# schreibfaul1/ESP32-Opus-Player

Hardware: AMD Instinct MI355X
Metric: decoded 48 kHz stereo frames/sec/GPU (x real-time); HBM GB/s vs roofline (higher is better)
Workload: dtype int32 fixed-point (int16/int32 with 64-bit products); 1 GPU; celt_fb_stereo_64k; streams_per_gpu=65536

## Files before the change

### esp32-opus-player_amd/csrc/og_celt_split.hpp

```cpp
#pragma once
#include <stddef.h>
#include "og_celt.hpp"

#undef OG_SYNC
#define OG_SYNC() OG_LSYNC()

namespace og {

constexpr int REC_BAND_WORDS = 4;
constexpr int REC_MAX_LEAVES = NBANDS * 2 * 16;
constexpr int REC_MAX_WORDS = NBANDS * (REC_BAND_WORDS + 2 * 33) + 3 * NBANDS + 1;

enum {
    RF_SILENCE = 1, RF_TRANSIENT = 2, RF_LM_SHIFT = 2 , RF_STEREO = 16, RF_SPREAD_SHIFT = 5 ,
    RF_DUAL = 128, RF_ANTI_COLLAPSE = 256, RF_RC_ERROR = 512, RF_TELL_OVERFLOW = 1024,
    RF_SKIP = 2048,
    RF_BAD_CELT = 4096
};
enum {
    BW_SIGN0 = 1, BW_SIGN1 = 2, BW_INV = 4, BW_SIGN = 8, BW_MID_FIRST = 16, BW_SWAP = 32,
    BW_THETA0 = 64, BW_THETA1 = 128,
    BW_TF_SHIFT = 8 , BW_FOLD0_SHIFT = 11 , BW_FOLD1_SHIFT = 16 ,
    BW_HAS_LOW = 1 << 21, BW_DUAL = 1 << 22, BW_DUAL_END = 1 << 23, BW_STEREO = 1 << 24,
    BW_DUAL_PRE = 1 << 25
};
enum {
    JW_NPVQ_SHIFT = 5 , JW_FIRST_SHIFT = 10 , JW_NEED_LOW = 1 << 20,
    LW_OFF_SHIFT = 8 , LW_B_SHIFT = 12 , LW_N_SHIFT = 16
};

struct SilkHandoff {
    alignas(128) i16 pcm[1920];
    u32 valid;
    u32 storage, end_offs, end_window;
    i32 nend_bits, nbits_total;
    u32 offs, rng, val, ext;
    i32 rem, error;
};
static_assert(sizeof(SilkHandoff) % 128 == 0 && offsetof(SilkHandoff, pcm) == 0, "handoff alignment");

struct ParseRec {
    i32 ret;
    u32 rng_final;
    u32 flags;
    i32 intensity, pf_pitch, pf_gain, pf_tapset, start;
    i32 n_leaves, n_words;
    u32 need_norm;
    i32 n_coef;
    i32 reserved[4];
    i16 bandE[2 * NBANDS];
    i16 pulses[NBANDS];
    u16 band_w[NBANDS];
    i8 tf_res[NBANDS];
    i8 pad[256 - 64 - 4 * NBANDS - 2 * NBANDS - 2 * NBANDS - NBANDS];
    struct Leaf {
        u32 idx;
        u32 geom;
        u32 aux;
        u32 pad;
    } leaf[REC_MAX_LEAVES];
    u32 words[(REC_MAX_WORDS + 64) / 64 * 64];
    i32 work_pulses[NBANDS];
    i32 work_pad[32 - NBANDS];
};
static_assert(offsetof(ParseRec, leaf) % 16 == 0 && offsetof(ParseRec, words) % 16 == 0 && offsetof(ParseRec, work_pulses) % 16 == 0 &&
              offsetof(ParseRec, work_pad) == offsetof(ParseRec, work_pulses) + 4 * NBANDS && NBANDS + 3 <= 32, "16-byte stores into the record");
static_assert(sizeof(ParseRec) % 16 == 0, "record alignment");

constexpr int FAST_MAX_LEAVES = 416;

#ifndef OG_PL_LANES
#define OG_PL_LANES (OG_NLANES >= 32 ? 32 : OG_NLANES)
#endif
#ifndef OG_PL_WAVES
#define OG_PL_WAVES 1
#endif
#ifdef OG_HOST_EMUL
#define OG_PWAVE 0
#define OG_PCOL OG_LANE
#else
#define OG_PWAVE ((int)(threadIdx.x >> 6))
#define OG_PCOL ((int)(threadIdx.x & 63))
#endif
#define OG_PL_FRAMES (OG_PL_LANES * OG_PL_WAVES)
struct ParseLds {
    i8 fine_quant[NBANDS][OG_PL_LANES];
    i8 tf_prio[NBANDS][OG_PL_LANES];
    union {
        i16 bandE[2 * NBANDS][OG_PL_LANES];
        struct {
            i16 offsets[NBANDS][OG_PL_LANES];
            u32 bw[NBANDS][OG_PL_LANES];
        } al;
        i32 stack[5][6][OG_PL_LANES];
    } u;
#ifdef OG_PL_PAD
    u8 pad_experiment[OG_PL_PAD];
#endif
};
#ifdef OG_PARSE_DYN_LDS
extern __shared__ __attribute__((aligned(16))) unsigned char og_dyn_lds[];
#define PLs (reinterpret_cast<ParseLds *>(og_dyn_lds))
#else
OG_LDS ParseLds PLs[OG_PL_WAVES];
#endif
#define PL PLs[OG_PWAVE]

struct ParseTabLds {
    i16 eband[NBANDS + 1], logn[NBANDS];
    u16 pulse_idx[105];
    u32 pulse_v[392];
    u8 pulse_bits[392], band_alloc[231], pulse_caps[168], log2_frac[24], eprob[336];
};
#ifdef OG_PARSE_DYN_LDS
#define PT (*reinterpret_cast<ParseTabLds *>(og_dyn_lds + sizeof(ParseLds) * OG_PL_WAVES))
#define OG_PARSE_LDS_BYTES (sizeof(ParseLds) * OG_PL_WAVES + sizeof(ParseTabLds))
#else
OG_LDS ParseTabLds PT;
#define OG_PARSE_LDS_BYTES 0
#endif
struct RomLds {
    static OG_MEMBER i32 eband(int i) { return PT.eband[i]; }
    static OG_MEMBER i32 logn(int i) { return PT.logn[i]; }
    static OG_MEMBER i32 pulse_idx(int i) { return PT.pulse_idx[i]; }
    static OG_MEMBER i32 pulse_bits(int i) { return PT.pulse_bits[i]; }
    static OG_MEMBER i32 band_alloc(int i) { return PT.band_alloc[i]; }
    static OG_MEMBER i32 pulse_caps(int i) { return PT.pulse_caps[i]; }
    static OG_MEMBER i32 log2_frac(int i) { return PT.log2_frac[i]; }
    static OG_MEMBER i32 eprob(int i) { return PT.eprob[i]; }
};
OG_DEV void parse_tables_load() {
    OG_FOR_LANES(i, NBANDS + 1) PT.eband[i] = rom_eband[i];
    OG_FOR_LANES(i, NBANDS) PT.logn[i] = rom_logn[i];
    OG_FOR_LANES(i, 105) PT.pulse_idx[i] = rom_pulse_idx[i];
    OG_FOR_LANES(i, 392) PT.pulse_bits[i] = rom_pulse_bits[i];
    OG_FOR_LANES(i, 392) PT.pulse_v[i] = rom_pulse_v[i];
    OG_FOR_LANES(i, 231) PT.band_alloc[i] = rom_band_alloc[i];
    OG_FOR_LANES(i, 168) PT.pulse_caps[i] = rom_pulse_caps[i];
    OG_FOR_LANES(i, 24) PT.log2_frac[i] = rom_log2_frac[i];
    OG_FOR_LANES(i, 336) PT.eprob[i] = rom_eprob[i];
    OG_FULL_SYNC();
}

struct TfResView {
    i8 *p;
    OG_MEMBER operator int() const { return (int)(i8)((u8)*p << 4) >> 4; }
    OG_MEMBER void operator=(int v) const { *p = (i8)((*p & 0xF0) | (v & 15)); }
};
struct FinePrioView {
    i8 *p;
    OG_MEMBER operator int() const { return (*p >> 4) & 1; }
    OG_MEMBER void operator=(int v) const { *p = (i8)((*p & ~0x10) | ((v & 1) << 4)); }
};
struct LaneArr {
    typedef RomLds Rom;
    i32 *pl;
    i16 *rest;
    i16 *pk;
    OG_MEMBER void energies_rest() const {
        for (int i = 0; i < 2 * NBANDS; i += 2)
            *reinterpret_cast<u32 *>(&rest[i]) = (u32)(u16)PL.u.bandE[i][OG_PCOL] | (u32)(u16)PL.u.bandE[i + 1][OG_PCOL] << 16;
        for (int i = 0; i < NBANDS; i++) PL.u.al.offsets[i][OG_PCOL] = 0;
    }
    OG_MEMBER void energies_back() const {
        u32 w[NBANDS];
        for (int i = 0; i < NBANDS; i++) w[i] = *reinterpret_cast<const u32 *>(&rest[2 * i]);
        for (int i = 0; i < NBANDS; i++) {
            PL.u.bandE[2 * i][OG_PCOL] = (i16)(w[i] & 0xffff);
            PL.u.bandE[2 * i + 1][OG_PCOL] = (i16)(w[i] >> 16);
        }
    }
    typedef u16 __attribute__((may_alias)) u16a;
    typedef i32 __attribute__((may_alias)) i32a;
    OG_MEMBER i32 &pulses(int i) const { return pl[i]; }
    OG_MEMBER i32a &alloc_bits(int i) const { return *reinterpret_cast<i32a *>(&PL.u.al.bw[i][OG_PCOL]); }
    OG_MEMBER void pulses_rest(int start, int end) const {
        i32 v[24];
        for (int i = 0; i < 24; i++) v[i] = (i >= start && i < end) ? (i32)PL.u.al.bw[i < NBANDS ? i : 0][OG_PCOL] : 0;
#ifdef OG_HOST_EMUL
        for (int i = 0; i < NBANDS; i++) pl[i] = v[i];
#else
        typedef i32 i32x4 __attribute__((ext_vector_type(4)));
        for (int i = 0; i < 24; i += 4) *reinterpret_cast<i32x4 *>(&pl[i]) = i32x4{v[i], v[i + 1], v[i + 2], v[i + 3]};
#endif
        for (int i = 0; i < NBANDS; i++) pk[i] = (i16)v[i];
    }
    OG_MEMBER i8 &fine_quant(int i) const { return PL.fine_quant[i][OG_PCOL]; }
    OG_MEMBER FinePrioView fine_prio(int i) const { return FinePrioView{&PL.tf_prio[i][OG_PCOL]}; }
    OG_MEMBER TfResView tf_res(int i) const { return TfResView{&PL.tf_prio[i][OG_PCOL]}; }
    OG_MEMBER i16 &offsets(int i) const { return PL.u.al.offsets[i][OG_PCOL]; }
    OG_MEMBER u16a &bits1(int i) const { return reinterpret_cast<u16a *>(&PL.u.al.bw[i][OG_PCOL])[0]; }
    OG_MEMBER u16a &bits2(int i) const { return reinterpret_cast<u16a *>(&PL.u.al.bw[i][OG_PCOL])[1]; }
    OG_MEMBER i16 &bandE(int i) const { return PL.u.bandE[i][OG_PCOL]; }
};

OG_DEV u32 pvq_u_rom(int a, int b) {
    const int lo = a < b ? a : b, hi = a < b ? b : a;
    return rom_pvq_u[lo * ROM_PVQ_COLS + hi];
}

struct RecWriter {
    ParseRec *rec;
    int nw, nl, ncoef = 0;
    int job = 0;
    OG_MEMBER void word(u32 w) {
        if (nw < REC_MAX_WORDS) rec->words[nw] = w;
        nw++;
    }
    OG_MEMBER int reserve() { return nw++; }
    OG_MEMBER void patch(int at, u32 w) {
        if (at < REC_MAX_WORDS) rec->words[at] = w;
    }
    OG_MEMBER void leaf(int x, int N, int K, int B, i32 gain, int off, u32 idx) {
        if (nl < REC_MAX_LEAVES) {
            const u32 geom = (u32)x | (u32)N << 11 | (u32)K << 19 | (u32)(B - 1) << 27;
            const u32 aux = (u32)(gain & 0xffff) | (u32)off << 16 | (u32)job << 20;
#ifdef OG_HOST_EMUL
            rec->leaf[nl].idx = idx; rec->leaf[nl].geom = geom; rec->leaf[nl].aux = aux; rec->leaf[nl].pad = 0;
#else
            typedef u32 u32x4 __attribute__((ext_vector_type(4)));
            *reinterpret_cast<u32x4 *>(&rec->leaf[nl]) = u32x4{idx, geom, aux, 0u};
#endif
        }
        nl++;
        ncoef += N;
    }
    OG_MEMBER int band_begin() { return nw = (nw + 3) & ~3; }
    OG_MEMBER void words4(u32 w0, u32 w1, u32 w2, u32 w3) {
        if (nw + 4 <= REC_MAX_WORDS) {
#ifdef OG_HOST_EMUL
            rec->words[nw] = w0; rec->words[nw + 1] = w1; rec->words[nw + 2] = w2; rec->words[nw + 3] = w3;
#else
            typedef u32 u32x4 __attribute__((ext_vector_type(4)));
            *reinterpret_cast<u32x4 *>(&rec->words[nw]) = u32x4{w0, w1, w2, w3};
#endif
        }
        nw += 4;
    }
};

OG_DEV int parse_tree(RcLane &rc, RecWriter &out, int band, i32 &remaining_bits, int x, int N, i32 b, int B, int LM, i32 gain,
                      int has_low, int silent) {
    int depth = 0, off = 0, n_fill = 0;
    const int jpos = out.reserve(), first_pvq = out.nl;
    for (;;) {
        OG_MARK(41);
        for (;;) {
            if (!(LM != -1 && b > pulse_cache_max<RomLds>(band, LM) + 12 && N > 2)) break;
            const int B0 = B;
            Split sc;
            i32 fill = 0;
            N >>= 1;
            LM -= 1;
            B = (B + 1) >> 1;
            compute_theta<RomLds>(rc, band, 0, 0, remaining_bits, sc, N, b, B, B0, LM, 0, fill);
            i32 delta = sc.delta;
            const int itheta = sc.itheta;
            if (B0 > 1 && (itheta & 0x3fff)) {
                if (itheta > 8192)
                    delta -= delta >> (4 - LM);
                else
                    delta = OG_MIN(0, delta + (N << BITRES >> (5 - LM)));
            }
            const i32 mbits = OG_MAX(0, OG_MIN(b, (b - delta) / 2));
            const i32 sbits = b - mbits;
            remaining_bits -= sc.qalloc;
            const int mid_first = mbits >= sbits;
            const int off_side = off + (B0 >> 1), silent_mid = silent | (itheta == 16384), silent_side = silent | (itheta == 0);
            i32 *F = &PL.u.stack[depth][0][OG_PCOL];
            F[0 * OG_PL_LANES] = x | N << 11 | (LM + 1) << 19 | B << 22 | mid_first << 27 | 1 << 28;
            F[1 * OG_PL_LANES] = mbits;
            F[2 * OG_PL_LANES] = sbits;
            F[3 * OG_PL_LANES] = remaining_bits;
            F[4 * OG_PL_LANES] = itheta | (mid_first ? off_side : off) << 16 | (mid_first ? silent_side : silent_mid) << 24;
            const i32 gain_mid = tr16(mul16_p15(gain, sc.imid)), gain_side = tr16(mul16_p15(gain, sc.iside));
            F[5 * OG_PL_LANES] = (gain_mid & 0xffff) | gain_side << 16;
            depth++;
            if (mid_first) {
                b = mbits;
                gain = gain_mid;
                silent = silent_mid;
            } else {
                x += N;
                b = sbits;
                gain = gain_side;
                off = off_side;
                silent = silent_side;
            }
        }
        {
            OG_MARK(42);
            int q = bits2pulses<RomLds>(band, LM, b), curr_bits = pulses2bits<RomLds>(band, LM, q);
            remaining_bits -= curr_bits;
            while (remaining_bits < 0 && q > 0) {
                remaining_bits += curr_bits;
                q--;
                curr_bits = pulses2bits<RomLds>(band, LM, q);
                remaining_bits -= curr_bits;
            }
            const int K = q ? get_pulses(q) : 0;
            OG_MARK(43);
            if (K)
                out.leaf(x, N, K, B, gain, off, rc_uint(rc, PT.pulse_v[pulse_cache<RomLds>(band, LM) + q]));
            else if (!silent) {
                out.word((u32)off << LW_OFF_SHIFT | (u32)(B - 1) << LW_B_SHIFT | (u32)N << LW_N_SHIFT);
                out.word((u32)x | (u32)(gain & 0xffff) << 11);
                n_fill++;
            }
        }
        OG_MARK(44);
        for (;;) {
            if (depth == 0) {
                OG_MARK(40);
                const int need_low = has_low && n_fill > 0;
                out.patch(jpos, (u32)n_fill | (u32)(out.nl - first_pvq) << JW_NPVQ_SHIFT | (u32)first_pvq << JW_FIRST_SHIFT |
                                    (need_low ? JW_NEED_LOW : 0));
                return need_low;
            }
            i32 *F = &PL.u.stack[depth - 1][0][OG_PCOL];
            const i32 w0 = F[0];
            const int mid_first = (w0 >> 27) & 1, stage = (w0 >> 28) & 3;
            if (stage == 1) {
                i32 mbits = F[1 * OG_PL_LANES], sbits = F[2 * OG_PL_LANES];
                const int itheta = F[4 * OG_PL_LANES] & 0x7fff;
                const i32 rebalance = (mid_first ? mbits : sbits) - (F[3 * OG_PL_LANES] - remaining_bits);
                if (mid_first) {
                    if (rebalance > 3 << BITRES && itheta != 0) sbits += rebalance - (3 << BITRES);
                } else {
                    if (rebalance > 3 << BITRES && itheta != 16384) mbits += rebalance - (3 << BITRES);
                }
                F[0] = (w0 & ~(3 << 28)) | 2 << 28;
                N = (w0 >> 11) & 255;
                LM = ((w0 >> 19) & 7) - 1;
                B = (w0 >> 22) & 31;
                x = (w0 & 2047) + (mid_first ? N : 0);
                b = mid_first ? sbits : mbits;
                gain = mid_first ? F[5 * OG_PL_LANES] >> 16 : (i32)(i16)F[5 * OG_PL_LANES];
                off = (F[4 * OG_PL_LANES] >> 16) & 15;
                silent = (F[4 * OG_PL_LANES] >> 24) & 1;
                break;
            }
            depth--;
        }
    }
}

OG_DEV u32 parse_all_bands(RcLane &rc, RecWriter &out, int start, int end, int C, int N_ch, int shortBlocks, int spread,
                           int dual_stereo, int intensity, i32 total_bits, i32 balance, int LM, int codedBands, int disable_inv) {
    const LaneArr a{out.rec->work_pulses, nullptr, nullptr};
    const int M = 1 << LM, B = shortBlocks ? M : 1;
    const int norm_offset = M * RomLds::eband(start);
    int lowband_offset = 0, update_lowband = 1;
    u32 need_norm = 0;
#ifdef OG_HOST_EMUL
    i32 p4[4] = {0, 0, 0, 0}, n4[4] = {0, 0, 0, 0};
    auto fetch4 = [&](int b, i32 *o) { for (int k = 0; k < 4; k++) o[k] = b + k < NBANDS ? a.pulses(b + k) : 0; };
    fetch4(start & ~3, n4);
#else
    typedef i32 i32x4p __attribute__((ext_vector_type(4)));
    i32x4p p4 = {0, 0, 0, 0}, n4 = *reinterpret_cast<const i32x4p *>(&a.pulses(start & ~3));
#endif
    for (int i = start; i < end; i++) {
        if (i == start || (i & 3) == 0) {
#ifdef OG_HOST_EMUL
            for (int k = 0; k < 4; k++) p4[k] = n4[k];
            fetch4((i & ~3) + 4, n4);
#else
            p4 = n4;
            n4 = *reinterpret_cast<const i32x4p *>(&a.pulses((i & ~3) + 4));
#endif
        }
        const i32 pulses_i = (i & 3) == 0 ? p4[0] : (i & 3) == 1 ? p4[1] : (i & 3) == 2 ? p4[2] : p4[3];
        const int eb0 = M * RomLds::eband(i), N = M * RomLds::eband(i + 1) - eb0;
        const int x = eb0, y = C == 2 ? N_ch + eb0 : -1;
        out.rec->band_w[i] = (u16)OG_MIN(out.band_begin(), REC_MAX_WORDS);
        const i32 tell = (i32)rc_tell_frac(rc);
        if (i != start) balance -= tell;
        i32 remaining_bits = total_bits - tell - 1, b;
        if (i <= codedBands - 1) {
            const i32 curr_balance = balance / OG_MIN(3, codedBands - i);
            b = OG_MAX(0, OG_MIN(16383, OG_MIN(remaining_bits + 1, pulses_i + curr_balance)));
        } else
            b = 0;
        const int tf_change = a.tf_res(i);
        if ((eb0 - N >= M * RomLds::eband(start) || i == start + 1) && (update_lowband || lowband_offset == 0)) lowband_offset = i;
        u32 w0 = (u32)(tf_change + 4) << BW_TF_SHIFT, w1 = (u32)eb0 << 11 | (u32)N << 22;
        int has_low = 0;
        u32 fold_bands = 0;
        if (lowband_offset != 0 && (spread != 3 || B > 1 || tf_change < 0)) {
            const int effective_lowband = OG_MAX(0, M * RomLds::eband(lowband_offset) - norm_offset - N);
            int fold_start = lowband_offset;
            while (M * RomLds::eband(--fold_start) > effective_lowband + norm_offset) {}
            int fold_end = lowband_offset - 1;
            while (++fold_end < i && M * RomLds::eband(fold_end) < effective_lowband + norm_offset + N) {}
            w0 |= BW_HAS_LOW | (u32)fold_start << BW_FOLD0_SHIFT | (u32)fold_end << BW_FOLD1_SHIFT;
            w1 |= (u32)effective_lowband;
            has_low = 1;
            fold_bands = (1u << fold_end) - (1u << fold_start);
        }
        if (dual_stereo) w0 |= BW_DUAL_PRE;
        if (dual_stereo && i == intensity) {
            dual_stereo = 0;
            w0 |= BW_DUAL_END;
        }
        if (dual_stereo) w0 |= BW_DUAL;
        u32 w2 = 0;
        if (N == 1) {
            for (int c = 0; c < (y >= 0 ? 2 : 1); c++) {
                if (remaining_bits >= 1 << BITRES) {
                    if (rc_bits(rc, 1)) w0 |= c ? BW_SIGN1 : BW_SIGN0;
                    remaining_bits -= 1 << BITRES;
                }
            }
            out.words4(w0, w1, 0, 0);
        } else {
            const int stereo = (y >= 0) && !dual_stereo;
            Split sc;
            sc.inv = 0; sc.imid = 0; sc.iside = 0; sc.delta = 0; sc.itheta = 0; sc.qalloc = 0;
            i32 bb = b, fill_unused = 0, mbits = 0, sbits = 0, rebal0 = 0;
            int n2case = 0, swap_c = 0, mid_first = 1, njobs = 1;
            if (stereo) {
                compute_theta<RomLds>(rc, i, intensity, disable_inv, remaining_bits, sc, N, bb, B, B, LM, 1, fill_unused);
                w0 |= BW_STEREO;
                if (sc.itheta == 0) w0 |= BW_THETA0;
                if (sc.itheta == 16384) w0 |= BW_THETA1;
                if (sc.itheta > 8192) w0 |= BW_SWAP;
                if (sc.inv) w0 |= BW_INV;
                w2 = (u32)(sc.imid & 0xffff) | (u32)sc.iside << 16;
                if (N == 2) {
                    n2case = 1;
                    mbits = bb;
                    sbits = 0;
                    if (sc.itheta != 0 && sc.itheta != 16384) sbits = 1 << BITRES;
                    mbits -= sbits;
                    swap_c = sc.itheta > 8192;
                    remaining_bits -= sc.qalloc + sbits;
                    if (sbits && rc_bits(rc, 1)) w0 |= BW_SIGN;
                } else {
                    mbits = OG_MAX(0, OG_MIN(bb, (bb - sc.delta) / 2));
                    sbits = bb - mbits;
                    remaining_bits -= sc.qalloc;
                    rebal0 = remaining_bits;
                    mid_first = mbits >= sbits;
                    njobs = 2;
                }
            } else if (dual_stereo)
                njobs = 2;
            if (mid_first) w0 |= BW_MID_FIRST;
            out.words4(w0, w1, w2, (u32)(u16)tr16(celt_sqrt(shl32(N, 22))));
            for (int jb = 0; jb < njobs; jb++) {
                int jx, jlow = has_low, jsilent = 0;
                i32 jbits, jgain = 32767;
                if (dual_stereo) {
                    jx = jb ? y : x;
                    jbits = b / 2;
                } else if (!stereo) {
                    jx = x;
                    jbits = b;
                } else if (n2case) {
                    jx = swap_c ? y : x;
                    jbits = mbits;
                } else {
                    const int is_mid = (jb == 0) == (mid_first != 0);
                    if (jb == 1) {
                        const i32 rebalance = (mid_first ? mbits : sbits) - (rebal0 - remaining_bits);
                        if (mid_first) {
                            if (rebalance > 3 << BITRES && sc.itheta != 0) sbits += rebalance - (3 << BITRES);
                        } else {
                            if (rebalance > 3 << BITRES && sc.itheta != 16384) mbits += rebalance - (3 << BITRES);
                        }
                    }
                    jx = is_mid ? x : y;
                    jbits = is_mid ? mbits : sbits;
                    jsilent = is_mid ? sc.itheta == 16384 : sc.itheta == 0;
                    if (!is_mid) {
                        jgain = sc.iside;
                        jlow = 0;
                    }
                }
                int Bj = B, N_B = (int)udiv((u32)N, (u32)B), tfc = tf_change;
                const int recombine = tfc > 0 ? tfc : 0;
                Bj >>= recombine;
                N_B <<= recombine;
                while ((N_B & 1) == 0 && tfc < 0) {
                    Bj <<= 1;
                    N_B >>= 1;
                    tfc++;
                }
                out.job = 2 * i + jb;
                if (parse_tree(rc, out, i, remaining_bits, jx, N, jbits, Bj, LM, jgain, jlow, jsilent)) need_norm |= fold_bands;
            }
        }
        balance += pulses_i + tell;
        update_lowband = b > (N << BITRES);
    }
    return need_norm;
}

OG_DEV void celt_parse_lane(StreamState *st, const u8 *payload, int len, int ch, ParseRec *rec, const SilkHandoff *handoff) {
    const LaneArr a{rec->work_pulses, rec->bandE, rec->pulses};
    const int CC = st->channels, C = ch, LM = 3, frame_size = 960, start = handoff ? 17 : 0, end = NBANDS;
    rec->start = start;
    rec->n_leaves = 0;
    rec->n_words = 0;
    if (len < 0 || len > 1275 || (handoff && !handoff->valid)) {
        rec->ret = BAD_ARG;
        rec->flags = RF_SKIP;
        return;
    }
    RcLane rc;
    rc_lane_attach(rc, payload, (u32)len);
    if (handoff) {
        rc.storage = handoff->storage; rc.end_offs = handoff->end_offs; rc.end_window = handoff->end_window;
        rc.nend_bits = handoff->nend_bits; rc.nbits_total = handoff->nbits_total; rc.offs = handoff->offs; rc.rng = handoff->rng;
        rc.val = handoff->val; rc.ext = handoff->ext; rc.rem = handoff->rem; rc.error = handoff->error;
        rc_lane_resume(rc);
    } else
        rc_init(rc, (u32)len);
    if (rc.storage <= 1) {
        rec->ret = CELT_BAD_ARG;
        rec->flags = RF_BAD_CELT;
        rec->rng_final = rc.rng;
        return;
    }
    const int disable_inv = CC == 1;
    for (int i = 0; i < 2 * NBANDS; i++) a.bandE(i) = st->celt.bandE[i];
    if (C == 1)
        for (int i = 0; i < NBANDS; i++) a.bandE(i) = (i16)OG_MAX((i32)a.bandE(i), (i32)a.bandE(NBANDS + i));
    for (int i = 0; i < NBANDS; i++) {
        a.fine_quant(i) = 0;
        a.fine_prio(i) = 0;
    }
    CeltHeader h;
    OG_MARK(20);
    celt_parse_header(a, rc, start, end, C, LM, h);
    a.energies_rest();
    RecWriter out;
    out.rec = rec;
    out.nw = 0;
    out.nl = 0;
    const int M = 1 << LM, N = M * 120;
    for (int i = 0; i < NBANDS; i++) rec->tf_res[i] = a.tf_res(i);
    OG_MARK(26);
    rec->need_norm = parse_all_bands(rc, out, start, end, C, N, h.transient ? M : 0, h.spread, h.dual_stereo, h.intensity,
                                     (i32)rc.storage * (8 << BITRES) - h.anti_collapse_rsv, h.balance, LM, h.codedBands, disable_inv);
    OG_MARK(27);
    int anti_collapse_on = 0;
    if (h.anti_collapse_rsv > 0) anti_collapse_on = (int)rc_bits(rc, 1);
    a.energies_back();
    energy_finalise(a, rc, start, end, (i32)rc.storage * 8 - rc_tell(rc), C);
    for (int i = 0; i < 2 * NBANDS; i++) rec->bandE[i] = a.bandE(i);
    u32 flags = (u32)LM << RF_LM_SHIFT | (u32)h.spread << RF_SPREAD_SHIFT;
    if (h.silence) flags |= RF_SILENCE;
    if (h.transient) flags |= RF_TRANSIENT;
    if (C == 2) flags |= RF_STEREO;
    if (h.dual_stereo) flags |= RF_DUAL;
    if (anti_collapse_on) flags |= RF_ANTI_COLLAPSE;
    if (rc.error || out.nw > REC_MAX_WORDS || out.nl > REC_MAX_LEAVES) flags |= RF_RC_ERROR;
    if (rc_tell(rc) > 8 * (i32)rc.storage) flags |= RF_TELL_OVERFLOW;
    rec->flags = flags;
    rec->ret = frame_size;
    rec->rng_final = rc.rng;
    rec->intensity = h.intensity;
    rec->pf_pitch = h.pf_pitch;
    rec->pf_gain = h.pf_gain;
    rec->pf_tapset = h.pf_tapset;
    rec->n_leaves = OG_MIN(out.nl, REC_MAX_LEAVES);
    rec->n_coef = out.ncoef;
    rec->n_words = OG_MIN(out.nw, REC_MAX_WORDS);
    for (int i = 0; i < 2 * NBANDS; i += 2) {
        i32 e[2];
        for (int k = 0; k < 2; k++) {
            const int band = i + k >= NBANDS ? i + k - NBANDS : i + k;
            e[k] = h.silence ? -28 * 1024 : (i32)a.bandE(C == 1 ? band : i + k);
            if (band < start || band >= end) e[k] = 0;
        }
        *reinterpret_cast<u32 *>(&st->celt.bandE[i]) = (u32)(u16)e[0] | (u32)(u16)e[1] << 16;
    }
}

#ifdef OG_HOST_EMUL
OG_DEV void rotate1_lane(i16 *xv, int x, int len, int stride, i32 c, i32 s) {
    const i32 ms = tr16(-s);
    for (int r = 0; r < stride; r++) {
        if (r < len - stride) {
            int i = r;
            i32 x1 = xv[x + i];
            for (; i < len - stride; i += stride) {
                const i32 x2 = xv[x + i + stride];
                xv[x + i] = (i16)pshr32(mul16(c, x1) + mul16(ms, x2), 15);
                x1 = tr16(pshr32(mul16(c, x2) + mul16(s, x1), 15));
            }
            xv[x + i] = (i16)x1;
        }
        const int last = len - 2 * stride - 1;
        if (last >= r) {
            int i = last - (last - r) % stride;
            i32 x2 = xv[x + i + stride];
            for (; i >= 0; i -= stride) {
                const i32 x1 = xv[x + i];
                xv[x + i + stride] = (i16)pshr32(mul16(c, x2) + mul16(s, x1), 15);
                x2 = tr16(pshr32(mul16(c, x1) + mul16(ms, x2), 15));
            }
            xv[x + r] = (i16)x2;
        }
    }
}
#else
OG_DEV i32 rot_dot2(u32 pair, u32 coef, i32 half) {
    i32 r;
    asm("v_dot2_i32_i16 %0, %1, %2, %3" : "=v"(r) : "v"(pair), "v"(coef), "v"(half));
    return r >> 15;
}
OG_DEV u32 rot_pack(i32 lo, i32 hi) { return __builtin_amdgcn_perm((u32)hi, (u32)lo, 0x05040100u); }
OG_DEV void rotate_chain(i16 *const p0, int r, int len, int stride, u32 k_a, u32 k_b) {
    const i32 half = 16384;
    int i = r, steps = 0;
    i32 x1 = p0[i];
    for (; i + 3 * stride < len - stride; i += 4 * stride, steps += 4) {
        const i32 e1 = p0[i + stride], e2 = p0[i + 2 * stride], e3 = p0[i + 3 * stride], e4 = p0[i + 4 * stride];
        u32 pk = rot_pack(x1, e1);
        const i32 o0 = rot_dot2(pk, k_a, half);
        x1 = rot_dot2(pk, k_b, half);
        pk = rot_pack(x1, e2);
        const i32 o1 = rot_dot2(pk, k_a, half);
        x1 = rot_dot2(pk, k_b, half);
        pk = rot_pack(x1, e3);
        const i32 o2 = rot_dot2(pk, k_a, half);
        x1 = rot_dot2(pk, k_b, half);
        pk = rot_pack(x1, e4);
        const i32 o3 = rot_dot2(pk, k_a, half);
        x1 = rot_dot2(pk, k_b, half);
        p0[i] = (i16)o0;
        p0[i + stride] = (i16)o1;
        p0[i + 2 * stride] = (i16)o2;
        p0[i + 3 * stride] = (i16)o3;
    }
    for (; i < len - stride; i += stride, steps++) {
        const u32 pk = rot_pack(x1, p0[i + stride]);
        p0[i] = (i16)rot_dot2(pk, k_a, half);
        x1 = rot_dot2(pk, k_b, half);
    }
    p0[i] = (i16)x1;
    if (steps >= 2) {
        i -= 2 * stride;
        i32 x2 = p0[i + stride];
        for (; i - 3 * stride >= 0; i -= 4 * stride) {
// ... 1437 lines not shown
```

### esp32-opus-player_amd/csrc/og_range.hpp

```cpp
#pragma once
#include "og_state.hpp"

namespace og {

OG_LDS FrameLds S;

struct Rc {
    u32 storage, end_offs, end_window;
    i32 nend_bits, nbits_total;
    u32 offs, rng, val, ext;
    i32 rem, error;
};
typedef u32 og_u32x4 __attribute__((ext_vector_type(4)));
struct RcLane : Rc {
    const u8 *buf;
#ifndef OG_HOST_EMUL
    const __attribute__((address_space(1))) og_u32x4 *chunks;
    const __attribute__((address_space(1))) u32 *words;
    u32 fshift, shift;
    i32 last_chunk, last_word;
    og_u32x4 f_cur, f_next;
    u32 b_cur, b_next;
    i32 f_idx, b_idx;
#endif
};

OG_DEV int rc_next_byte(Rc &rc) { return rc.offs < rc.storage ? S.pkt[rc.offs++] : 0; }
OG_DEV int rc_next_byte_end(Rc &rc) {
    return rc.end_offs < rc.storage ? S.pkt[rc.storage - ++rc.end_offs] : 0;
}
#ifdef OG_HOST_EMUL
OG_DEV void rc_lane_attach(RcLane &rc, const u8 *buf, u32 len) {
    rc.buf = buf;
    (void)len;
}
OG_DEV void rc_lane_resume(RcLane &rc) {}
OG_DEV int rc_next_byte(RcLane &rc) { return rc.offs < rc.storage ? rc.buf[rc.offs++] : 0; }
OG_DEV int rc_next_byte_end(RcLane &rc) { return rc.end_offs < rc.storage ? rc.buf[rc.storage - ++rc.end_offs] : 0; }
#else
OG_DEV u32 rc_lane_word(const RcLane &rc, i32 w) { return (w >= 0 && w <= rc.last_word) ? rc.words[w] : 0u; }
OG_DEV og_u32x4 rc_lane_chunk(const RcLane &rc, i32 w) { return (w >= 0 && w <= rc.last_chunk) ? rc.chunks[w] : og_u32x4{0u, 0u, 0u, 0u}; }
OG_DEV void rc_lane_attach(RcLane &rc, const u8 *buf, u32 len) {
    rc.buf = buf;
    const unsigned long long a = (unsigned long long)buf;
    rc.chunks = (const __attribute__((address_space(1))) og_u32x4 *)(a & ~15ull);
    rc.words = (const __attribute__((address_space(1))) u32 *)(a & ~3ull);
    rc.fshift = (u32)(a & 15ull);
    rc.shift = (u32)(a & 3ull);
    rc.last_chunk = len ? (i32)((rc.fshift + len - 1) >> 4) : -1;
    rc.last_word = len ? (i32)((rc.shift + len - 1) >> 2) : -1;
    rc.f_idx = 0;
    rc.f_cur = rc_lane_chunk(rc, 0);
    rc.f_next = rc_lane_chunk(rc, 1);
    rc.b_idx = rc.last_word;
    rc.b_cur = rc_lane_word(rc, rc.b_idx);
    rc.b_next = rc_lane_word(rc, rc.b_idx - 1);
}
OG_DEV void rc_lane_resume(RcLane &rc) {
    rc.f_idx = (i32)((rc.offs + rc.fshift) >> 4);
    rc.f_cur = rc_lane_chunk(rc, rc.f_idx);
    rc.f_next = rc_lane_chunk(rc, rc.f_idx + 1);
    rc.b_idx = rc.end_offs < rc.storage ? (i32)((rc.storage - rc.end_offs - 1 + rc.shift) >> 2) : rc.last_word;
    rc.b_cur = rc_lane_word(rc, rc.b_idx);
    rc.b_next = rc_lane_word(rc, rc.b_idx - 1);
}
OG_DEV int rc_next_byte(RcLane &rc) {
    if (rc.offs >= rc.storage) return 0;
    const u32 pos = rc.offs++ + rc.fshift;
    const i32 w = (i32)(pos >> 4);
    if (w != rc.f_idx) {
        rc.f_cur = rc.f_next;
        rc.f_idx = w;
        rc.f_next = rc_lane_chunk(rc, w + 1);
    }
    const bool up = (pos & 8u) != 0;
    const u32 lo = up ? rc.f_cur.z : rc.f_cur.x, hi = up ? rc.f_cur.w : rc.f_cur.y;
    return (int)__builtin_amdgcn_perm(hi, lo, 0x0c0c0c00u | (pos & 7u));
}
OG_DEV int rc_next_byte_end(RcLane &rc) {
    if (rc.end_offs >= rc.storage) return 0;
    const u32 pos = rc.storage - ++rc.end_offs + rc.shift;
    const i32 w = (i32)(pos >> 2);
    if (w != rc.b_idx) {
        rc.b_cur = rc.b_next;
        rc.b_idx = w;
        rc.b_next = rc_lane_word(rc, w - 1);
    }
    return (int)((rc.b_cur >> (8 * (pos & 3))) & 255u);
}
#endif

template <class R>
OG_DEV void rc_renorm(R &rc) {
    while (rc.rng <= (1u << 23)) {
        rc.nbits_total += 8;
        rc.rng <<= 8;
        int sym = rc.rem;
        rc.rem = rc_next_byte(rc);
        sym = (sym << 8 | rc.rem) >> 1;
        rc.val = ((rc.val << 8) + (255u & ~(u32)sym)) & 0x7FFFFFFFu;
    }
}

template <class R>
OG_DEV void rc_init(R &rc, u32 len) {
    rc.storage = len;
    rc.end_offs = 0;
    rc.end_window = 0;
    rc.nend_bits = 0;
    rc.nbits_total = 9;
    rc.offs = 0;
    rc.rng = 128;
    rc.rem = rc_next_byte(rc);
    rc.val = rc.rng - 1 - (rc.rem >> 1);
    rc.ext = 0;
    rc.error = 0;
    rc_renorm(rc);
}

template <class R>
OG_DEV i32 rc_tell(const R &rc) { return rc.nbits_total - ilog(rc.rng); }

template <class R>
OG_DEV u32 rc_tell_frac(const R &rc) {
    u32 nbits = (u32)rc.nbits_total << 3;
    int l = ilog(rc.rng);
    u32 r = rc.rng >> (l - 16);
    u32 b = (r >> 12) - 8;
    u32 corr = b == 0 ? 35733u : b == 1 ? 38967u : b == 2 ? 42495u : b == 3 ? 46340u
             : b == 4 ? 50535u : b == 5 ? 55109u : b == 6 ? 60097u : 65535u;
    b += r > corr;
    return nbits - (u32)((l << 3) + b);
}

template <class R>
OG_DEV u32 rc_decode(R &rc, u32 ft) {
    rc.ext = rc.rng / ft;
    u32 s = rc.val / rc.ext;
    return ft - OG_MIN(s + 1, ft);
}

template <class R>
OG_DEV u32 rc_decode_bin(R &rc, unsigned bits) {
    rc.ext = rc.rng >> bits;
    u32 s = rc.val / rc.ext, top = 1u << bits;
    return top - OG_MIN(s + 1u, top);
}

template <class R>
OG_DEV void rc_update(R &rc, u32 fl, u32 fh, u32 ft) {
    u32 s = rc.ext * (ft - fh);
    rc.val -= s;
    rc.rng = fl > 0 ? rc.ext * (fh - fl) : rc.rng - s;
    rc_renorm(rc);
}

template <class R>
OG_DEV int rc_bit_logp(R &rc, unsigned logp) {
    u32 r = rc.rng, d = rc.val, s = r >> logp;
    int ret = d < s;
    if (!ret) rc.val = d - s;
    rc.rng = ret ? s : r - s;
    rc_renorm(rc);
    return ret;
}

template <class R>
OG_DEV int rc_icdf(R &rc, const u8 *icdf, unsigned ftb) {
    u32 s = rc.rng, d = rc.val, r = s >> ftb, t;
    int ret = -1;
    do {
        t = s;
        s = r * icdf[++ret];
    } while (d < s);
    rc.val = d - s;
    rc.rng = t - s;
    rc_renorm(rc);
    return ret;
}

#ifndef OG_HOST_EMUL
OG_DEV int rc_icdf(Rc &rc, const u8 *icdf, unsigned ftb) {
    const u32 d = rc.val, r = rc.rng >> ftb;
    const u32 s_l = r * (u32)icdf[OG_LANE];
    const u64 hit = __ballot(d >= s_l);
    const int ret = (int)__builtin_ctzll(hit);
    const u32 s = (u32)__builtin_amdgcn_readlane((int)s_l, ret);
    const u32 t = ret ? (u32)__builtin_amdgcn_readlane((int)s_l, ret - 1) : rc.rng;
    rc.val = d - s;
    rc.rng = t - s;
    rc_renorm(rc);
    return ret;
}
#endif

template <class R>
OG_DEV u32 rc_bits(R &rc, unsigned bits) {
    u32 window = rc.end_window;
    int available = rc.nend_bits;
    if ((u32)available < bits) {
        do {
            window |= (u32)rc_next_byte_end(rc) << available;
            available += 8;
        } while (available <= 24);
    }
    u32 ret = window & ((1u << bits) - 1u);
    rc.end_window = window >> bits;
    rc.nend_bits = available - (int)bits;
    rc.nbits_total += bits;
    return ret;
}

template <class R>
OG_DEV u32 rc_uint(R &rc, u32 ft_in) {
    ft_in--;
    int ftb = ilog(ft_in);
    if (ftb > 8) {
        ftb -= 8;
        u32 ft = (ft_in >> ftb) + 1;
        u32 s = rc_decode(rc, ft);
        rc_update(rc, s, s + 1, ft);
        u32 t = s << ftb | rc_bits(rc, ftb);
        if (t <= ft_in) return t;
        rc.error = 1;
        return ft_in;
    }
    ft_in++;
    u32 s = rc_decode(rc, ft_in);
    rc_update(rc, s, s + 1, ft_in);
    return s;
}

template <class R>
OG_DEV int rc_laplace(R &rc, u32 fs, int decay) {
    int val = 0;
    u32 fl = 0, fm = rc_decode_bin(rc, 15);
    if (fm >= fs) {
        val++;
        fl = fs;
        fs = ((32768u - 32u - fs) * (u32)(16384 - decay) >> 15) + 1;
        while (fs > 1 && fm >= fl + 2 * fs) {
            fs *= 2;
            fl += fs;
            fs = ((fs - 2) * (u32)decay) >> 15;
            fs += 1;
            val++;
        }
        if (fs <= 1) {
            int di = (int)((fm - fl) >> 1);
            val += di;
            fl += 2 * di;
        }
        if (fm < fl + fs)
            val = -val;
        else
            fl += fs;
    }
    rc_update(rc, fl, OG_MIN(fl + fs, 32768u), 32768u);
    return val;
}

}
```

Before: 42.94 million frames/s.

## Specialize lane-parallel split theta decode and compact the parse recursion stack

Replaces the generic compute_theta call in the band-split tree with a lane-specialized split_theta_lane. It decodes the triangular theta distribution in closed form using a float-based integer sqrt, where the generic path searches for it. The per-lane LDS recursion stack shrinks from 5x6 to 4x5 words: the first-child choice is resolved at push time, so the pop needs no stage field or mid/side branching. A branch-reduced rc_uint overload for RcLane is also added. The goal is less divergence and LDS footprint in the parse kernel, at the risk of bit-exactness errors in the sqrt-based inverse and a reduced maximum recursion depth.

```diff
diff --git a/esp32-opus-player_amd/csrc/og_celt_split.hpp b/esp32-opus-player_amd/csrc/og_celt_split.hpp
--- a/esp32-opus-player_amd/csrc/og_celt_split.hpp
+++ b/esp32-opus-player_amd/csrc/og_celt_split.hpp
@@ -92,7 +92,7 @@
             i16 offsets[NBANDS][OG_PL_LANES];
             u32 bw[NBANDS][OG_PL_LANES];
         } al;
-        i32 stack[5][6][OG_PL_LANES];
+        i32 stack[4][5][OG_PL_LANES];
     } u;
 #ifdef OG_PL_PAD
     u8 pad_experiment[OG_PL_PAD];
@@ -239,6 +239,64 @@
     }
 };
 
+OG_DEV u32 isqrt24(u32 val) {
+    u32 g = (u32)__builtin_sqrtf((float)val);
+    g -= g * g > val;
+    g += (g + 1) * (g + 1) <= val;
+    return g;
+}
+
+OG_DEV void split_theta_lane(RcLane &rc, int band, Split &sc, int N, i32 &b, int B0, int LM) {
+    int itheta = 0;
+    const int pulse_cap = RomLds::logn(band) + LM * (1 << BITRES);
+    const int offset = (pulse_cap >> 1) - 4;
+    const int qn = compute_qn(N, b, offset, pulse_cap, 0);
+    const u32 tell = rc_tell_frac(rc);
+    if (qn != 1) {
+        const bool uni = B0 > 1;
+        const int h = qn >> 1;
+        const int ftb = uni ? OG_MAX(ilog((u32)qn) - 8, 0) : 0;
+        const u32 ft = uni ? (u32)(qn >> ftb) + 1 : (u32)((h + 1) * (h + 1));
+        const u32 fm = rc_decode(rc, ft);
+        const bool low = fm < (u32)(h * (h + 1) >> 1);
+        const u32 root = isqrt24(8 * (low ? fm : ft - fm - 1) + 1);
+        const int it = low ? (int)((root - 1) >> 1) : (int)((2u * (u32)(qn + 1) - root) >> 1);
+        const int fs_t = low ? it + 1 : qn + 1 - it;
+        const u32 fl_t = low ? (u32)(it * (it + 1) >> 1) : ft - (u32)(fs_t * (fs_t + 1) >> 1);
+        const u32 fl = uni ? fm : fl_t, fs = uni ? 1u : (u32)fs_t;
+        rc_update(rc, fl, fl + fs, ft);
+        itheta = uni ? (int)fm : it;
+        if (ftb) {
+            const u32 t = fm << ftb | rc_bits(rc, (unsigned)ftb);
+            if (t > (u32)qn) rc.error = 1;
+            itheta = (int)OG_MIN(t, (u32)qn);
+        }
+        itheta = (int)udiv((u32)(itheta * 16384), (u32)qn);
+    }
+    const int qalloc = (int)(rc_tell_frac(rc) - tell);
+    b -= qalloc;
+    int imid, iside, delta;
+    if (itheta == 0) {
+        imid = 32767;
+        iside = 0;
+        delta = -16384;
+    } else if (itheta == 16384) {
+        imid = 0;
+        iside = 32767;
+        delta = 16384;
+    } else {
+        imid = bitexact_cos(itheta);
+        iside = bitexact_cos(16384 - itheta);
+        delta = frac_mul16((N - 1) << 7, bitexact_log2tan(iside, imid));
+    }
+    sc.inv = 0;
+    sc.imid = imid;
+    sc.iside = iside;
+    sc.delta = delta;
+    sc.itheta = itheta;
+    sc.qalloc = qalloc;
+}
+
 OG_DEV int parse_tree(RcLane &rc, RecWriter &out, int band, i32 &remaining_bits, int x, int N, i32 b, int B, int LM, i32 gain,
                       int has_low, int silent) {
     int depth = 0, off = 0, n_fill = 0;
@@ -249,11 +307,10 @@
             if (!(LM != -1 && b > pulse_cache_max<RomLds>(band, LM) + 12 && N > 2)) break;
             const int B0 = B;
             Split sc;
-            i32 fill = 0;
             N >>= 1;
             LM -= 1;
             B = (B + 1) >> 1;
-            compute_theta<RomLds>(rc, band, 0, 0, remaining_bits, sc, N, b, B, B0, LM, 0, fill);
+            split_theta_lane(rc, band, sc, N, b, B0, LM);
             i32 delta = sc.delta;
             const int itheta = sc.itheta;
             if (B0 > 1 && (itheta & 0x3fff)) {
@@ -267,14 +324,17 @@
             remaining_bits -= sc.qalloc;
             const int mid_first = mbits >= sbits;
             const int off_side = off + (B0 >> 1), silent_mid = silent | (itheta == 16384), silent_side = silent | (itheta == 0);
+            const i32 gain_mid = tr16(mul16_p15(gain, sc.imid)), gain_side = tr16(mul16_p15(gain, sc.iside));
+#ifdef OG_HOST_EMUL
+            if (x + N >= 2048 || N > 255 || LM + 1 > 7 || B > 31 || off_side > 15) __builtin_trap();
+#endif
             i32 *F = &PL.u.stack[depth][0][OG_PCOL];
-            F[0 * OG_PL_LANES] = x | N << 11 | (LM + 1) << 19 | B << 22 | mid_first << 27 | 1 << 28;
-            F[1 * OG_PL_LANES] = mbits;
-            F[2 * OG_PL_LANES] = sbits;
+            F[0 * OG_PL_LANES] = (i32)((u32)(mid_first ? x + N : x) | (u32)N << 11 | (u32)(LM + 1) << 19 | (u32)B << 22 |
+                                       (u32)(mid_first ? off_side : off) << 27 | (u32)(mid_first ? silent_side : silent_mid) << 31);
+            F[1 * OG_PL_LANES] = mid_first ? mbits : sbits;
+            F[2 * OG_PL_LANES] = mid_first ? sbits : mbits;
             F[3 * OG_PL_LANES] = remaining_bits;
-            F[4 * OG_PL_LANES] = itheta | (mid_first ? off_side : off) << 16 | (mid_first ? silent_side : silent_mid) << 24;
-            const i32 gain_mid = tr16(mul16_p15(gain, sc.imid)), gain_side = tr16(mul16_p15(gain, sc.iside));
-            F[5 * OG_PL_LANES] = (gain_mid & 0xffff) | gain_side << 16;
+            F[4 * OG_PL_LANES] = ((mid_first ? gain_side : gain_mid) & 0xffff) | (itheta != (mid_first ? 0 : 16384)) << 16;
             depth++;
             if (mid_first) {
                 b = mbits;
@@ -309,40 +369,27 @@
             }
         }
         OG_MARK(44);
-        for (;;) {
-            if (depth == 0) {
-                OG_MARK(40);
-                const int need_low = has_low && n_fill > 0;
-                out.patch(jpos, (u32)n_fill | (u32)(out.nl - first_pvq) << JW_NPVQ_SHIFT | (u32)first_pvq << JW_FIRST_SHIFT |
-                                    (need_low ? JW_NEED_LOW : 0));
-                return need_low;
-            }
-            i32 *F = &PL.u.stack[depth - 1][0][OG_PCOL];
-            const i32 w0 = F[0];
-            const int mid_first = (w0 >> 27) & 1, stage = (w0 >> 28) & 3;
-            if (stage == 1) {
-                i32 mbits = F[1 * OG_PL_LANES], sbits = F[2 * OG_PL_LANES];
-                const int itheta = F[4 * OG_PL_LANES] & 0x7fff;
-                const i32 rebalance = (mid_first ? mbits : sbits) - (F[3 * OG_PL_LANES] - remaining_bits);
-                if (mid_first) {
-                    if (rebalance > 3 << BITRES && itheta != 0) sbits += rebalance - (3 << BITRES);
-                } else {
-                    if (rebalance > 3 << BITRES && itheta != 16384) mbits += rebalance - (3 << BITRES);
-                }
-                F[0] = (w0 & ~(3 << 28)) | 2 << 28;
-                N = (w0 >> 11) & 255;
-                LM = ((w0 >> 19) & 7) - 1;
-                B = (w0 >> 22) & 31;
-                x = (w0 & 2047) + (mid_first ? N : 0);
-                b = mid_first ? sbits : mbits;
-                gain = mid_first ? F[5 * OG_PL_LANES] >> 16 : (i32)(i16)F[5 * OG_PL_LANES];
-                off = (F[4 * OG_PL_LANES] >> 16) & 15;
-                silent = (F[4 * OG_PL_LANES] >> 24) & 1;
-                break;
-            }
+        if (depth == 0) break;
+        {
             depth--;
-        }
-    }
+            const i32 *F = &PL.u.stack[depth][0][OG_PCOL];
+            const u32 w0 = (u32)F[0];
+            const i32 w4 = F[4 * OG_PL_LANES];
+            const i32 rebalance = F[1 * OG_PL_LANES] - (F[3 * OG_PL_LANES] - remaining_bits);
+            b = F[2 * OG_PL_LANES] + ((rebalance > 3 << BITRES && (w4 >> 16)) ? rebalance - (3 << BITRES) : 0);
+            x = (int)(w0 & 2047);
+            N = (int)(w0 >> 11) & 255;
+            LM = (int)((w0 >> 19) & 7) - 1;
+            B = (int)(w0 >> 22) & 31;
+            off = (int)(w0 >> 27) & 15;
+            silent = (int)(w0 >> 31);
+            gain = (i32)(i16)w4;
+        }
+    }
+    OG_MARK(40);
+    const int need_low = has_low && n_fill > 0;
+    out.patch(jpos, (u32)n_fill | (u32)(out.nl - first_pvq) << JW_NPVQ_SHIFT | (u32)first_pvq << JW_FIRST_SHIFT | (need_low ? JW_NEED_LOW : 0));
+    return need_low;
 }
 
 OG_DEV u32 parse_all_bands(RcLane &rc, RecWriter &out, int start, int end, int C, int N_ch, int shortBlocks, int spread,
diff --git a/esp32-opus-player_amd/csrc/og_range.hpp b/esp32-opus-player_amd/csrc/og_range.hpp
--- a/esp32-opus-player_amd/csrc/og_range.hpp
+++ b/esp32-opus-player_amd/csrc/og_range.hpp
@@ -229,6 +229,19 @@
     u32 s = rc_decode(rc, ft_in);
     rc_update(rc, s, s + 1, ft_in);
     return s;
+}
+
+OG_DEV u32 rc_uint(RcLane &rc, u32 ft_in) {
+    ft_in--;
+    const int ftb = OG_MAX(ilog(ft_in) - 8, 0);
+    const u32 ft = (ft_in >> ftb) + 1;
+    const u32 s = rc_decode(rc, ft);
+    rc_update(rc, s, s + 1, ft);
+    if (ftb == 0) return s;
+    const u32 t = s << ftb | rc_bits(rc, (unsigned)ftb);
+    if (t <= ft_in) return t;
+    rc.error = 1;
+    return ft_in;
 }
 
 template <class R>
```

Result: faster. 43.66 million frames/s, median of 6 (+1.7%).
